# sidiso/surfh

Measured on AMD Instinct MI355X. Metric: CG-iterations/sec (forward+adjoint) on 251x251x4000 cube, higher is better.
Workload: dtype f32 (storage and accumulation; products as 2-piece fp16 splits -- 3 products per fp32 product, 1 on the far tails of the spectral response -- on the 16-bit matrix cores, in the spectral-blur GEMM and in the DFT passes)

## Files before the change

include/surfh_amd.h:

```cpp
#ifndef SURFH_AMD_H
#define SURFH_AMD_H

#include <stdint.h>

#ifdef __cplusplus
extern "C" {
#endif

typedef struct surfh_plan surfh_plan;

typedef struct {
    int32_t wslice_start, wslice_stop;
    int32_t n_pointings;
    int32_t n_slit;
    int32_t n_lambda_out;
    int32_t n_alpha_out;
    int32_t srf;
    int32_t na, nb;
    int32_t alpha0;
    int32_t n_alpha_slit;
    int32_t n_beta_slit;
    const int32_t *slit_beta0;
    const double *slit_weights;
    const int32_t *grid_i0;
// ... 130 lines not shown

int surfh_profile_enable(surfh_plan *plan, int32_t on);
int surfh_profile_filter(surfh_plan *plan, const char *prefix);
int32_t surfh_profile_count(surfh_plan *plan);
int surfh_profile_get(surfh_plan *plan, int32_t i, const char **name, int64_t *launches, double *ms);
int surfh_profile_reset(surfh_plan *plan);

int64_t surfh_debug_copy(surfh_plan *plan, const char *which, float *out, int64_t capacity);
int surfh_debug_dims(surfh_plan *plan, const char *which, int64_t dims[4]);

int surfh_gemm_selftest(int32_t device, int32_t M, int32_t N, int32_t K, int32_t split_k,
                        const float *A, const float *B, float *C);
int surfh_gemm_selftest_ksteps(int64_t near_far[2]);
int32_t surfh_klist_classify(const float *B, int32_t n, int32_t k, int64_t ldb, int32_t perm_p, int32_t perm_lin,
                             int32_t *records, int64_t capacity);

typedef struct surfh_tst surfh_tst;
int surfh_tst_create(int32_t n_alpha, int32_t n_beta, int32_t n_lambda, int32_t n_templates, const double *templates,
                     const int32_t *voxels, int64_t n_voxels, const float *S, int32_t device, surfh_tst **out);
int surfh_tst_destroy(surfh_tst *t);
int surfh_tst_forward(surfh_tst *t, const float *maps, float *cube);
int surfh_tst_adjoint(surfh_tst *t, const float *cube, float *maps);
int surfh_tst_fwadj(surfh_tst *t, const float *maps, float *out);
const char *surfh_tst_last_error(void);

int surfh_shepard(int32_t n_seg, const int64_t *pt_off, const float *pt_alpha, const float *pt_lambda,
                  const float *pt_value, const int32_t *n_alpha, const int32_t *n_lambda, int32_t separable,
                  const float *q_alpha, const float *q_lambda, const float *inv_alpha_res, const float *inv_lambda_res,
                  float p, float alpha, float pixel_cutoff, float epsilon, float *out, int32_t *neighbours,
                  int32_t device_ptrs, void *stream, float *kernel_ms);
// ... 14 lines not shown
```

surfh_amd/_lib.py:

```python
from __future__ import annotations

import ctypes as C
import os

import numpy as np

_HERE = os.path.dirname(os.path.abspath(__file__))
LIB_PATH = os.path.join(_HERE, "libsurfh_amd.so")

c_float_p = C.POINTER(C.c_float)
c_double_p = C.POINTER(C.c_double)
c_int32_p = C.POINTER(C.c_int32)
CG_CALLBACK = C.CFUNCTYPE(C.c_int, C.c_void_p, C.c_int32, c_double_p, c_float_p)
c_uint8_p = C.POINTER(C.c_uint8)


class ChannelDesc(C.Structure):
    _fields_ = [
        ("wslice_start", C.c_int32), ("wslice_stop", C.c_int32),
        ("n_pointings", C.c_int32), ("n_slit", C.c_int32), ("n_lambda_out", C.c_int32),
        ("n_alpha_out", C.c_int32), ("srf", C.c_int32), ("na", C.c_int32), ("nb", C.c_int32),
        ("alpha0", C.c_int32), ("n_alpha_slit", C.c_int32), ("n_beta_slit", C.c_int32),
        ("slit_beta0", c_int32_p), ("slit_weights", c_double_p),
        ("grid_i0", c_int32_p), ("grid_i1", c_int32_p), ("grid_y0", c_double_p), ("grid_y1", c_double_p),
# ... 13 lines not shown
        ("exact", C.c_int32),
    ]


EXPORTS = [
    "surfh_last_error", "surfh_version", "surfh_plan_create", "surfh_plan_destroy", "surfh_isize", "surfh_osize",
    "surfh_stream", "surfh_forward", "surfh_adjoint", "surfh_adjoint_ref", "surfh_fwadj", "surfh_forward_dev",
    "surfh_adjoint_dev", "surfh_adjoint_ref_dev", "surfh_fwadj_dev", "surfh_wct_forward", "surfh_wct_adjoint",
    "surfh_wct_fwadj", "surfh_wct_expsol", "surfh_tst_create", "surfh_tst_destroy", "surfh_tst_forward",
    "surfh_tst_adjoint", "surfh_tst_fwadj", "surfh_tst_last_error", "surfh_cg", "surfh_cg_cb", "surfh_mmmg", "surfh_mmmg_huber", "surfh_huber_prior_dev", "surfh_huber_curv_dev", "surfh_mmmg_huber_vox", "surfh_huber_vox_prior_dev", "surfh_huber_vox_curv_dev", "surfh_mmmg_huber_planes", "surfh_huber_planes_prior_dev", "surfh_huber_planes_curv_dev", "surfh_cg_planes", "surfh_mmmg_planes", "surfh_cg_planes_cb", "surfh_mmmg_planes_cb", "surfh_cg_planes_begin_dev", "surfh_cg_planes_step_dev", "surfh_cg_planes_rr", "surfh_maps_to_cube", "surfh_cube_to_maps", "surfh_normal_dev",
    "surfh_prior_add_dev", "surfh_spec_supported", "surfh_spec_size", "surfh_to_spec_dev", "surfh_from_spec_dev", "surfh_forward_spec_dev",
    "surfh_adjoint_spec_dev", "surfh_normal_spec_dev", "surfh_prior_spec_add_dev", "surfh_set_prior", "surfh_set_data_weights", "surfh_set_data_weights_dev", "surfh_has_data_weights", "surfh_dot_dev", "surfh_cg_step_dev", "surfh_cg_dir_dev", "surfh_cg_iter_dev", "surfh_residual_dev",
    "surfh_cg_begin_dev", "surfh_cg_iter_nosync_dev", "surfh_cg_xupdate_nosync_dev", "surfh_cg_refresh_nosync_dev", "surfh_cg_trace",
    "surfh_profile_enable", "surfh_profile_filter", "surfh_profile_count", "surfh_profile_get", "surfh_profile_reset", "surfh_debug_copy",
    "surfh_debug_dims", "surfh_gemm_selftest", "surfh_gemm_selftest_ksteps", "surfh_klist_classify",
    "surfh_shepard", "surfh_shepard_last_error", "surfh_spectral_median", "surfh_nmf_cd", "surfh_templates_last_error",
]

_lib = None


def load():
    global _lib
    if _lib is not None:
        return _lib
    if not os.path.exists(LIB_PATH):
        raise RuntimeError(f"{LIB_PATH} not found: run `python -c 'import __graft_entry__ as g; g.build()'` "
                           "(the HIP path has no CPU fallback)")
    L = C.CDLL(LIB_PATH)
    vp = C.c_void_p
# ... 65 lines not shown
    L.surfh_cg_iter_nosync_dev.argtypes = [vp, vp, vp, vp, vp, C.c_int64]
    L.surfh_cg_xupdate_nosync_dev.argtypes = [vp, vp, vp, vp, C.c_int64]
    L.surfh_cg_refresh_nosync_dev.argtypes = [vp, vp, vp, vp, vp, C.c_int64]
    L.surfh_cg_trace.argtypes = [vp, c_double_p, C.c_int32]; L.surfh_cg_trace.restype = C.c_int32
    L.surfh_profile_enable.argtypes = [vp, C.c_int32]
    L.surfh_profile_filter.argtypes = [vp, C.c_char_p]
    L.surfh_profile_count.argtypes = [vp]; L.surfh_profile_count.restype = C.c_int32
    L.surfh_profile_get.argtypes = [vp, C.c_int32, C.POINTER(C.c_char_p), C.POINTER(C.c_int64), c_double_p]
    L.surfh_profile_reset.argtypes = [vp]
    L.surfh_debug_copy.argtypes = [vp, C.c_char_p, c_float_p, C.c_int64]; L.surfh_debug_copy.restype = C.c_int64
    L.surfh_debug_dims.argtypes = [vp, C.c_char_p, C.POINTER(C.c_int64)]
    L.surfh_gemm_selftest.argtypes = [C.c_int32] * 5 + [c_float_p, c_float_p, c_float_p]
    L.surfh_gemm_selftest_ksteps.argtypes = [C.POINTER(C.c_int64)]
    L.surfh_klist_classify.argtypes = [c_float_p, C.c_int32, C.c_int32, C.c_int64, C.c_int32, C.c_int32, C.POINTER(C.c_int32), C.c_int64]
    L.surfh_klist_classify.restype = C.c_int32
    L.surfh_shepard.argtypes = [C.c_int32, C.POINTER(C.c_int64), vp, vp, vp, c_int32_p, c_int32_p, C.c_int32, vp, vp,
                                c_float_p, c_float_p, C.c_float, C.c_float, C.c_float, C.c_float, vp, vp, C.c_int32, vp,
                                c_float_p]
    L.surfh_shepard_last_error.restype = C.c_char_p
    L.surfh_spectral_median.argtypes = [c_float_p, c_float_p, C.c_int64, C.c_int64, C.c_int32, C.c_int32, C.c_int32]
    L.surfh_nmf_cd.argtypes = [c_float_p, C.c_int64, C.c_int64, C.c_int32, c_int32_p, c_float_p, c_float_p, C.c_int32,
                               C.c_double, c_int32_p, c_double_p, c_double_p, c_double_p, C.c_int32, c_float_p]
    L.surfh_templates_last_error.restype = C.c_char_p
    _lib = L
    return L


def check(rc: int, exc=RuntimeError):
    if rc != 0:
        raise exc(load().surfh_last_error().decode("utf-8", "replace"))
# ... 82 lines not shown
```

surfh_amd/csrc/dft_h2.h:

```cpp
#pragma once
#include <hip/hip_runtime.h>

constexpr int DFT_H2_KT = 8;
constexpr size_t DFT_H2_IMAGE_HALFS = (size_t)2 * 2 * DFT_H2_KT * 128 * 16;

struct DftH2Args {
    int kind = 0;
    const float *src = nullptr;
    long ldb = 0, sB = 0;
    int Kn = 0;
    float *dst = nullptr;
    long ldc = 0, sC = 0;
    float e[4] = {1.f, 0.f, 0.f, 1.f};
    float e_alt[4] = {1.f, 0.f, 0.f, 1.f};
    int Rn = 0, rvalid = 0;
    int KP = 0;
    int N = 0, batch = 1;
    const float *mhat = nullptr, *tpl = nullptr;
    int T = 0, LP = 0;
    long PL = 0, KBP = 0;
    int mix_l0 = 0;
    float mhat_self = 1.f, mhat_pair = 1.f;
    int mix_Nb = 0;
    const int *vlist = nullptr;
    int nvalid = 0;
    const int *ktab = nullptr, *rtab = nullptr;
    int tabLP = 0;
};

struct DftH2AdjMix {
    const float *hsrc = nullptr;
    long ldh = 0, sH = 0;
    const float *tpl = nullptr;
    int T = 0, LPt = 0;
    float *mpart = nullptr;
    int nslot = 0;
    int kt0 = 0;
    float out_self = 1.f, out_pair = 1.f;
    int Nb = 0;
    const float *prior_src = nullptr;
// ... 12 lines not shown
```

surfh_amd/csrc/dft_h2.hip:

```cpp
#include "dft_h2.h"
#include "lds_attr.h"
#include <cmath>
#include <cstring>

typedef float f32x16 __attribute__((ext_vector_type(16)));
typedef float f32x2 __attribute__((ext_vector_type(2)));
typedef unsigned u32x2 __attribute__((ext_vector_type(2)));
typedef _Float16 f16x8 __attribute__((ext_vector_type(8)));

#ifndef H2_EXP
#define H2_EXP 0
#endif

namespace {

constexpr int BK = 16, RS = 16;
constexpr int PIECE = 128 * RS;
constexpr int KT = DFT_H2_KT;
constexpr int IMG_HALFS = (int)DFT_H2_IMAGE_HALFS;
constexpr int MIX_ROWS = 256;
constexpr size_t LDS_IMG = (size_t)IMG_HALFS * 2;
constexpr size_t LDS_MIX = (size_t)2 * MIX_ROWS * 2 * sizeof(float4);
#ifndef H2_WAVES
#define H2_WAVES 8
// ... 173 lines not shown

    if (MIX) {
        if (ntw > 0) {
            const int t0_ = NWAVES * s0 + wave;
            const int kb0 = g.batch > 1 ? t0_ / tilesX : ((t0_ % tilesX) * TNW) / g.LP;
            H2_MIXTAB(kb0);
        }
    }
    __syncthreads();
    if (ntw <= 0) return;

    const int *vl = g.vlist;
#define H2_RT(vt_) (vl ? NWAVES * vl[(vt_) >> 3] + ((vt_) & 7) : (vt_))
    int vt = NWAVES * s0 + wave;
    const int vtend = vt + NWAVES * ntw;
    int tile = H2_RT(vt);
    int e = 0, en = 0;

    H2_LSETUP(tile);
    H2_LOAD(0);
    H2_FSETUP(tile);
    H2_FOLD(0);
    {
        int p;
        H2_MAXEXP(p);
        e = E_TARGET - p;
    }
    split8h(x0, e, c0h, c0l);
    split8h(x1, e, c1h, c1l);
    H2_LOAD(1);
    while (true) {
        asm volatile("" : "+v"(hv));
#pragma unroll
        for (int i = 0; i < 4; ++i)
#pragma unroll
            for (int r = 0; r < 16; ++r) acc1[i][r] = acc2[i][r] = 0.f;
        const bool more = vt + NWAVES < vtend;
        const int next = more ? H2_RT(vt + NWAVES) : tile;
        const int chunk_ = g.tabLP ? (int)(((long)(tile % tilesX) * TNW % g.tabLP) >> 7) : 0;
        const int nkt = g.ktab ? g.ktab[chunk_] : nk;
        const int mtn = g.rtab ? (g.rtab[chunk_] + 31) / 32 : 4;
        for (int kt = 0; kt + 1 < nkt; ++kt) {
            H2_MFMA(0, kt, acc1, c0h, c0l);
            H2_FOLD(kt + 1);
            int p;
            H2_MAXEXP(p);
            const bool need = p + e > E_LIMIT;
            en = need ? E_TARGET - p : e;
            const int d = en - e;
            if (kt + 2 < nkt) {
                H2_LOAD(kt + 2);
            } else if (more) {
                H2_LSETUP(next);
                H2_LOAD(0);
            }
// ... 45 lines not shown
                            __builtin_amdgcn_raw_buffer_store_b64(__builtin_bit_cast(u32x2, v2), W0, (int)lo, (int)sk0, 0);
                        } else {
                            __builtin_amdgcn_raw_buffer_store_b32(__float_as_uint(e0 * a1 + e1 * a2), W0, (int)lo, (int)sk0, 0);
                            if (row >= 1 && 2 * row != g.Rn)
                                __builtin_amdgcn_raw_buffer_store_b32(__float_as_uint(e2 * a1 + e3 * a2), W0, (int)lm, (int)sm0, 0);
                        }
                    }
                    const unsigned st = ((r & 3) == 3) ? 5u * ldc4 : ldc4;
                    sk0 += st; sm0 -= st;
                }
            }
        }
        if (!more) break;
        e = en;
        tile = next;
        vt += NWAVES;
    }
}


__device__ __forceinline__ float wave_max(float m) {
#define H2_DPPMAX(ctrl_) m = fmaxf(m, __builtin_bit_cast(float, __builtin_amdgcn_update_dpp(0, __builtin_bit_cast(int, m), ctrl_, 0xF, 0xF, false)))
    H2_DPPMAX(0xB1);
    H2_DPPMAX(0x4E);
    H2_DPPMAX(0x141);
    H2_DPPMAX(0x140);
#undef H2_DPPMAX
    unsigned u = __float_as_uint(m);
    auto s16 = __builtin_amdgcn_permlane16_swap(u, u, false, false);
    m = fmaxf(m, fmaxf(__uint_as_float(s16[0]), __uint_as_float(s16[1])));
    u = __float_as_uint(m);
    auto s32 = __builtin_amdgcn_permlane32_swap(u, u, false, false);
// ... 342 lines not shown
    const int mix_rows = g.Kn > g.KP ? g.Kn : g.KP;
    if (g.mhat && (g.kind != 0 || g.LP % 128 || g.T < 1 || g.T > 4 || mix_rows > MIX_ROWS || !g.tpl)) return (int)hipErrorInvalidValue;
    static int cus_of[64] = {0};
    int dev = 0;
    if (hipGetDevice(&dev) != hipSuccess || dev < 0 || dev >= 64) return (int)hipErrorInvalidDevice;
    if (!cus_of[dev]) {
        int cus = 0;
        if (hipDeviceGetAttribute(&cus, hipDeviceAttributeMultiprocessorCount, dev) != hipSuccess) return (int)hipErrorInvalidDevice;
        cus_of[dev] = cus;
    }
    const int tnw = g.kind == 0 ? 16 : 32;
    long NT = (long)(g.N / tnw) * g.batch;
    long NS = (NT + NWAVES - 1) / NWAVES;
    if (NS >= 2147483647L / NWAVES) return (int)hipErrorInvalidValue;
    if ((g.ktab || g.rtab) && (g.tabLP < 128 || g.tabLP % 128)) return (int)hipErrorInvalidValue;
    if (g.vlist) {
        if (NT % NWAVES || g.nvalid < 1 || g.nvalid > NS) return (int)hipErrorInvalidValue;
        NS = g.nvalid;
        NT = NS * NWAVES;
    }
    dim3 grid((unsigned)(NS < cus_of[dev] ? NS : cus_of[dev]));
    const uint4 *im = reinterpret_cast<const uint4 *>(img);
    static unsigned long long d0 = 0, d1 = 0, d2 = 0, d3 = 0;
    if (g.mhat) {
        if (int e = ensure_dynamic_lds(dft_h2_kernel<0, true>, LDS_IMG + LDS_MIX, d3)) return e;
        hipLaunchKernelGGL((dft_h2_kernel<0, true>), grid, dim3(NTHREADS), LDS_IMG + LDS_MIX, stream, g, im, kA, (int)NS, NT);
    } else if (g.kind == 0) {
        if (int e = ensure_dynamic_lds(dft_h2_kernel<0, false>, LDS_IMG, d0)) return e;
        hipLaunchKernelGGL((dft_h2_kernel<0, false>), grid, dim3(NTHREADS), LDS_IMG, stream, g, im, kA, (int)NS, NT);
    } else if (g.kind == 1) {
// ... 60 lines not shown
```

surfh_amd/csrc/plan.hip:

```cpp
#include <hip/hip_runtime.h>

#include <algorithm>
#include <array>
#include <cfloat>
#include <cmath>
#include <cstdarg>
#include <cstdio>
#include <cstring>
#include <map>
#include <string>
#include <vector>

#include "../../include/surfh_amd.h"
#include "dft_h2.h"
#include "dft_ct.h"
#include "gemm_f32.h"
#include "kernels.h"

namespace {

thread_local std::string g_err;

int fail(const char *fmt, ...) {
    char buf[1024];
// ... 109 lines not shown
    unsigned short *h2img = nullptr;
    bool ct = false, ilv = false;
    DftCtPlan ctA, ctB;
    int ax_a = 0, ax_b = 0;
    int a_lo = 0, a_hi = 0, b_lo = 0, b_hi = 0;
    float *ycol_adj = nullptr;
    const float *spec_in = nullptr;
    float *spec_out = nullptr;
    const float *spec_prior_src = nullptr;
    float spec_mu = 1.f, spec_prior_mu = 0.f;
    float *adjmix_part = nullptr;
    int *otf_vlist = nullptr, *otf_kbstart = nullptr;
    int otf_nvalid = 0;
    int *otf_tabs = nullptr;
    float *ycol_mix = nullptr;
    int h2kA[3] = {0, 0, 0};
    float *io_x = nullptr, *io_y = nullptr, *io_cube = nullptr, *hth = nullptr, *mhat2 = nullptr;
    float *gcube = nullptr;
    std::vector<Channel> ch;
    long isize = 0, osize = 0;
    float *dw = nullptr, *dwy = nullptr;
    float *cg_x = nullptr, *cg_r = nullptr, *cg_d = nullptr, *cg_q = nullptr, *cg_b = nullptr, *cg_y = nullptr, *cg_qm = nullptr, *cg_dd = nullptr;
    float *cg_hg = nullptr;
    double *dscal = nullptr, *dscratch = nullptr;
    double *cg_hist = nullptr;
    int cg_hist_n = 0;
    double *pl_sc = nullptr;
    double *pl_hsc = nullptr;
    float *pl_x = nullptr;
    double pl_mu = 1.0, pl_mu_reg = 0.0;
// ... 601 lines not shown
        Prof pr(p, "gemm_dft_cols_inv");
        LAUNCH_OK(gemm32(p, p->stream, g));
    }
    GemmArgs h;
    h.A0 = p->GiT; h.lda = 2 * p->KBP;
    h.B0 = p->ycol; h.B1 = p->ycol + (long)p->NAP * p->KBP * LP; h.ksplitB = p->KBP; h.ldb = LP; h.sB = p->KBP * LP;
    h.C = dst; h.ldc = p->NAP * LP; h.sC = LP;
    h.M = p->NBP; h.N = (int)LP; h.K = 2 * p->KBP; h.batch = p->NAP;
    {
        Prof pr(p, "gemm_dft_rows_inv");
        LAUNCH_OK(gemm32(p, p->stream, h));
    }
    return 0;
}

int otf_support(surfh_plan *p, const surfh_config *cfg) {
    const bool on = [] { const char *e = getenv("SURFH_OTF_SUPPORT"); return !(e && e[0] == '0'); }();
    if (cfg->exact & 2) return 0;
    if (!on || !cfg->sotf || !p->ilv || p->T < 1 || !p->fuse_mix || p->LP % 128) return 0;
    const int nkb = p->Nb / 2 + 1, nch = (int)(p->LP / 128);
    std::vector<int> bmax(nch, -1), amaxk(nch, -1);
    std::vector<double> km(nkb), kam(p->Na);
    for (int l = 0; l < p->Lown; ++l) {
        if (p->planes[l] < 0) continue;
        std::fill(km.begin(), km.end(), 0.0);
        std::fill(kam.begin(), kam.end(), 0.0);
        double amax = 0.0;
        const double *pl = cfg->sotf + (size_t)p->planes[l] * p->Na * nkb * 2;
        for (int a = 0; a < p->Na; ++a)
            for (int k = 0; k < nkb; ++k) {
                const double re = pl[((size_t)a * nkb + k) * 2], im = pl[((size_t)a * nkb + k) * 2 + 1], m2 = re * re + im * im;
                if (m2 > km[k]) km[k] = m2;
                if (m2 > kam[a]) kam[a] = m2;
            }
        for (int k = 0; k < nkb; ++k) amax = std::max(amax, km[k]);
        const double thr = amax * std::ldexp(1.0, -48);
        int b = -1;
        for (int k = 0; k < nkb; ++k)
            if (km[k] > thr) b = k;
        bmax[l / 128] = std::max(bmax[l / 128], b);
        int af = -1;
        for (int a = 0; a < p->Na; ++a)
            if (kam[a] > thr) af = std::max(af, std::min(a, p->Na - a));
        amaxk[l / 128] = std::max(amaxk[l / 128], af);
    }
    std::vector<int> vlist, kbstart(nkb + 1, 0);
    for (int kb = 0; kb < nkb; ++kb) {
        kbstart[kb] = (int)vlist.size();
        for (int j = 0; j < nch; ++j)
            if (kb <= bmax[j]) vlist.push_back(kb * nch + j);
    }
    kbstart[nkb] = (int)vlist.size();
    if (vlist.empty() || (long)vlist.size() == (long)nkb * nch) return 0;
    const size_t nyc = (size_t)2 * p->NAP * p->KBP * p->LP;
    if (dev_upload(&p->otf_vlist, vlist) || dev_upload(&p->otf_kbstart, kbstart) || dev_alloc(&p->ycol_mix, nyc)) return 1;
    if (hipMemset(p->ycol_mix, 0, nyc * sizeof(float)) != hipSuccess) return fail("memset failed");
    p->otf_nvalid = (int)vlist.size();
    std::vector<int> tabs((size_t)(p->ct ? 4 : 3) * nch);
    for (int j = 0; j < nch; ++j) {
        if (p->ct) {
            const int ja = (std::max(amaxk[j], 0) + p->ctA.R - 1) / p->ctA.R, jb = (std::max(bmax[j], 0) + p->ctB.R - 1) / p->ctB.R;
            tabs[j] = std::min(std::max(ja / 16 + 1, 2), p->ctA.KT);
            tabs[nch + j] = std::min(std::max(jb / 16 + 1, 2), p->ctB.KT);
            tabs[2 * nch + j] = bmax[j];
            tabs[3 * nch + j] = amaxk[j];
            continue;
        }
        tabs[j] = std::min(std::max((amaxk[j] + 16) / 16, 2), p->KPa / 16);
        tabs[nch + j] = std::min(std::max((bmax[j] + 16) / 16, 2), p->KPb / 16);
        tabs[2 * nch + j] = bmax[j] + 1;
    }
    const bool ranges = [] { const char *e = getenv("SURFH_OTF_RANGES"); return !(e && e[0] == '0'); }();
    if (ranges && dev_upload(&p->otf_tabs, tabs)) return 1;
    return 0;
}

int rfft2_lam_h2(surfh_plan *p, const float *src, float *dst, float *madj = nullptr, bool acols = false, int which = 3) {
    const long LP = p->LP;
    const int ha = p->Na / 2 + 1, hb = p->Nb / 2 + 1;
    const bool sub = acols && p->ycol_adj && p->a_hi > p->a_lo;
    float *const yc = sub ? p->ycol_adj : p->ycol;
    const int a0 = sub ? p->a_lo : 0, na = sub ? p->a_hi - p->a_lo : p->Na;
    DftH2Args g;
    g.kind = 1; g.src = src + (long)a0 * LP; g.ldb = p->NAP * LP; g.Kn = p->Nb;
    g.dst = yc + 2 * (long)a0 * LP; g.ldc = 2 * p->NAP * LP; g.e[0] = 1.f; g.e[3] = -1.f; g.rvalid = hb;
    g.KP = p->KPb; g.N = (int)(na * LP);
    if (madj && p->otf_vlist && p->ycol_mix && p->otf_tabs) { g.rtab = p->otf_tabs + 2 * (LP / 128); g.tabLP = (int)LP; }
    if (which & 1) {
        Prof pr(p, "dft_h2_rows_fwd");
        LAUNCH_OK(launch_dft_h2(p->stream, g, p->h2img + 2 * DFT_H2_IMAGE_HALFS, p->h2kA[2]));
    }
    if (!(which & 2)) return 0;
    DftH2Args h;
    h.kind = 0; h.src = yc; h.ldb = 2 * LP; h.sB = 2 * p->NAP * LP; h.Kn = p->Na;
    h.dst = dst; h.ldc = 2 * p->KBP * LP; h.sC = 2 * LP; h.Rn = p->Na; h.rvalid = ha;
    h.KP = p->KPa; h.N = (int)LP; h.batch = hb;
    h.e[0] = 1.f; h.e[1] = 1.f; h.e[2] = 1.f; h.e[3] = -1.f;
    h.e_alt[0] = 1.f; h.e_alt[1] = -1.f; h.e_alt[2] = 1.f; h.e_alt[3] = 1.f;
// ... 24 lines not shown
int irfft2_lam_h2(surfh_plan *p, const float *src, float *dst, bool mix, bool acols = false, int which = 3) {
    const long LP = p->LP;
    const int ha = p->Na / 2 + 1, hb = p->Nb / 2 + 1;
    DftH2Args g;
    g.kind = 0; g.src = src; g.ldb = 2 * p->KBP * LP; g.Kn = p->Na;
    g.dst = p->ycol; g.ldc = 2 * p->KBP * LP; g.Rn = p->Na; g.rvalid = ha;
    g.KP = p->KPa; g.N = (int)(hb * LP);
    g.e[0] = 1.f; g.e[1] = -1.f; g.e[2] = 1.f; g.e[3] = 1.f;
    g.e_alt[0] = 1.f; g.e_alt[1] = 1.f; g.e_alt[2] = 1.f; g.e_alt[3] = -1.f;
    if (mix) { g.mhat = p->mhat; g.tpl = p->tpl; g.T = p->T; g.LP = (int)p->LP; g.PL = p->PL; g.KBP = p->KBP; }
    if (mix && p->spec_in) { g.mhat = p->spec_in; g.mhat_self = 1.f; g.mhat_pair = 0.70710678118654752f; g.mix_Nb = p->Nb; }
    const bool supp = mix && p->otf_vlist && p->ycol_mix && p->adjmix_part;
    float *const yc = supp ? p->ycol_mix : p->ycol;
    if (supp) { g.vlist = p->otf_vlist; g.nvalid = p->otf_nvalid; g.dst = yc; }
    if (supp && p->otf_tabs) { g.ktab = p->otf_tabs; g.tabLP = (int)LP; }
    if (which & 2) {
        Prof pr(p, mix ? "dft_h2_cols_inv_mix" : "dft_h2_cols_inv");
        LAUNCH_OK(launch_dft_h2(p->stream, g, p->h2img, p->h2kA[0]));
    }
    if (!(which & 1)) return 0;
    const bool sub = acols && p->a_hi > p->a_lo;
    const int a0 = sub ? p->a_lo : 0, na = sub ? p->a_hi - p->a_lo : p->Na;
    DftH2Args h;
    h.kind = 2; h.src = yc + (long)a0 * 2 * p->KBP * LP; h.ldb = 2 * LP; h.sB = 2 * p->KBP * LP;
    h.dst = dst + (long)a0 * LP; h.ldc = p->NAP * LP; h.sC = LP;
    h.e[0] = 1.f; h.e[1] = -1.f; h.e[2] = 1.f; h.e[3] = 1.f; h.Rn = p->Nb; h.rvalid = hb;
    h.KP = p->KPb; h.N = (int)LP; h.batch = na;
    if (supp && p->otf_tabs) { h.ktab = p->otf_tabs + LP / 128; h.tabLP = (int)LP; }
    {
        Prof pr(p, "dft_h2_rows_inv");
        LAUNCH_OK(launch_dft_h2(p->stream, h, p->h2img + DFT_H2_IMAGE_HALFS, p->h2kA[1]));
    }
    return 0;
}

int rfft2_lam_ct(surfh_plan *p, const float *src, float *dst, bool acols = false, bool lists = false, int which = 3) {
    const long LP = p->LP;
    const int hb = p->Nb / 2 + 1;
    const bool sub = acols && p->ycol_adj && p->a_hi > p->a_lo;
    float *const yc = sub ? p->ycol_adj : p->ycol;
    const int a0 = sub ? p->a_lo : 0, na = sub ? p->a_hi - p->a_lo : p->Na;
    DftCtArgs g;
    g.R = p->ctB.R; g.M = p->ctB.M; g.loader = DFT_CT_PLAIN; g.epi = DFT_CT_HSEP; g.sgn = -1.f;
// ... 410 lines not shown
int surfh_version(void) { return 100; }

int surfh_plan_destroy(surfh_plan *p) {
    if (!p) return 0;
    hipSetDevice(p->dev);
    if (p->stream) hipStreamSynchronize(p->stream);
    for (float *v : {p->sotf, p->tpl, p->mhat, p->spec, p->ycol, p->cube, p->ycol_maps, p->maps_pad, p->Fi, p->Gi, p->Gf,
                     p->Ff, p->GiT, p->GfT, p->Cma, p->Sma, p->Gc, p->Gs, p->Cf, p->Sf, p->io_cube, p->hth, p->mhat2, p->gcube, p->io_x, p->io_y, p->cg_x, p->cg_r, p->cg_d, p->cg_q, p->cg_b, p->cg_y, p->cg_qm, p->cg_dd, p->cg_hg})
        hipFree(v);
    hipFree(p->h2img);
    if (p->ctB.img != p->ctA.img) dft_ct_plan_destroy(&p->ctB);
    else p->ctB = DftCtPlan();
    dft_ct_plan_destroy(&p->ctA);
    hipFree(p->adjmix_part);
    hipFree(p->otf_vlist);
    hipFree(p->otf_kbstart);
    hipFree(p->otf_tabs);
    hipFree(p->ycol_mix);
    hipFree(p->ycol_adj);
    hipFree(p->dscal);
    hipFree(p->dscratch);
    hipFree(p->cg_hist);
    hipFree(p->pl_sc);
    hipFree(p->pl_hsc);
    for (float *v : p->pn_v) hipFree(v);
    hipFree(p->dw);
    hipFree(p->dwy);
    hipFree(p->pn_sc);
    hipFree(p->pn_part);
    for (auto &c : p->ch) {
// ... 100 lines not shown

    {
        const char *eh = getenv("SURFH_DFT_H2"), *ec = getenv("SURFH_DFT_CT"), *ed = getenv("SURFH_DFT_DENSE");
        const bool h2_on = !(eh && eh[0] == '0'), ct_on = !(ec && ec[0] == '0');
        auto axis = [&](int n) {
            if (h2_on && dft_h2_supported(n, n, p->NAP, p->KBP, p->LP)) return 1;
            if (ct_on && dft_ct_factor(n, nullptr, nullptr)) return 2;
            return 0;
        };
        p->ax_a = axis(p->Na);
        p->ax_b = axis(p->Nb);
        p->ilv = !cfg->verify && !(ed && ed[0] == '1') && p->LP % 128 == 0 && p->ax_a && p->ax_b;
        if (!p->ilv) p->ax_a = p->ax_b = 0;
        p->h2 = p->ilv && p->ax_a == 1 && p->ax_b == 1;
        p->ct = p->ilv && !p->h2;
    }
    {
        const int nkb = p->Nb / 2 + 1;
        const size_t nsp = (size_t)2 * p->PL * LP;
        if (dev_alloc(&p->sotf, nsp)) return bail(1);
        if (hipMemset(p->sotf, 0, nsp * sizeof(float)) != hipSuccess) return bail(fail("memset failed"));
        std::vector<float> row((size_t)2 * p->KBP * LP);
        for (int a = 0; a < p->Na; ++a) {
            std::fill(row.begin(), row.end(), 0.f);
            for (int l = 0; l < p->Lown; ++l) {
                if (p->planes[l] < 0) continue;
                const double *src = cfg->sotf ? cfg->sotf + ((size_t)p->planes[l] * p->Na + a) * nkb * 2 : nullptr;
                for (int k = 0; k < nkb; ++k) {
                    const float vr = src ? (float)src[2 * k] : 1.f, vi = src ? (float)src[2 * k + 1] : 0.f;
                    if (p->ilv) {
// ... 234 lines not shown
                    size_t n = 1;
                    while (n < (size_t)SCATTER_G && r + n < h.rows.size() && h.dst[r + n] == h.dst[r + n - 1] + p->LP) ++n;
                    runs.push_back({r, n});
                    r += n;
                }
                if (upload_groups(h, runs, &mask, &c.adjT, SCATTER_G, &ranges)) return bail(1);
            }
            c.adjT_host = HostEll();
            if (dev_upload(&c.adjT.rmw, mask) || dev_upload(&c.adjT.rng, ranges)) return bail(1);
            c.adjT.t.rng = c.adjT.rng;
            const char *ea = getenv("SURFH_SCATTER_RMW_ALL");
            if (!(ea && ea[0] == '1')) c.adjT.t.rmw = c.adjT.rmw;
            c.adjT.host_dst.clear();
            c.adjT.host_dst.shrink_to_fit();
        }
        if (exact_ok && !p->ch.empty()) {
            const size_t ncube = (size_t)p->NBP * p->NAP * p->LP;
            if (dev_alloc(&p->gcube, ncube)) return bail(1);
            if (hipMemset(p->gcube, 0, ncube * sizeof(float)) != hipSuccess) return bail(fail("memset failed"));
        } else {
            for (auto &c : p->ch) {
                c.adjT.t.rng = nullptr;
                c.adjT.g.rng = nullptr;
            }
        }
    }
    if (dev_alloc(&p->io_x, (size_t)p->isize) || dev_alloc(&p->io_y, (size_t)p->osize) || dev_alloc(&p->cg_y, (size_t)p->osize) ||
        dev_alloc(&p->dscal, 16) || dev_alloc(&p->dscratch, std::max((size_t)1024, launch_huber_vox_scratch_doubles())))
        return bail(1);
    if (hipDeviceSynchronize() != hipSuccess) return bail(fail("device error during plan creation: %s", hipGetErrorString(hipGetLastError())));
// ... 1241 lines not shown
            dims[0] = p->ch[c].LinP; dims[1] = p->ch[c].shift; dims[2] = p->ch[c].nbs; dims[3] = p->ch[c].Lin;
        } else {
            Channel &ch = p->ch[c];
            if (ch.Xs16) {
                if (launch_dequant_f16x2(p->stream, ch.Xs16, (long)ch.NP * ch.K, ch.bscale, ch.Xs, ch.NP, ch.K, ch.LinP,
                                         (ch.LinP + 1023) / 1024))
                    return fail("dequant launch failed");
                if (hipStreamSynchronize(p->stream) != hipSuccess) return fail("dequant failed");
            }
            *ptr = p->ch[c].Xs; dims[0] = p->ch[c].NP; dims[1] = p->ch[c].bsum ? 1 : p->ch[c].nbs; dims[2] = p->ch[c].LinP;
        }
    } else if (w == "range") {
        dims[0] = p->a_lo; dims[1] = p->a_hi; dims[2] = p->b_lo; dims[3] = p->b_hi;
    } else if (w == "otf") {
        dims[0] = p->otf_vlist ? p->otf_nvalid : (long)(p->Nb / 2 + 1) * (p->LP / 128); dims[1] = (long)(p->Nb / 2 + 1) * (p->LP / 128);
    } else if (w == "ksteps") {
        for (auto &c : p->ch)
            for (int i = 0; i < 4; ++i) dims[i] += c.ksteps[i];
        for (int i = 0; i < 4; ++i) dims[i] -= 1;
    } else if (w == "info") {
        dims[0] = p->lo; dims[1] = p->hi; dims[2] = p->Lown; dims[3] = (int64_t)p->segs.size();
    } else {
        return fail("unknown debug buffer '%s'", w.c_str());
    }
    return 0;
}

int surfh_debug_dims(surfh_plan *p, const char *which, int64_t dims[4]) {
    if (!p) return fail("null plan");
    const float *ptr;
// ... 16 lines not shown
    return n;
}

int32_t surfh_klist_classify(const float *B, int32_t n, int32_t k, int64_t ldb, int32_t perm_p, int32_t perm_lin, int32_t *records,
                             int64_t capacity) {
    if (!B || !records || n < 1 || k < 32 || k % 32 || ldb < k) return -fail("surfh_klist_classify: bad arguments");
    if (perm_p && ((perm_p != 1 && perm_p != 2 && perm_p != 4 && perm_p != 8) || perm_lin < 1 || perm_lin % (256 / perm_p) || n % perm_lin))
        return -fail("surfh_klist_classify: bad tile shape");
    std::vector<int> kl;
    int stride = 0;
    long nn = 0, nf = 0;
    build_klist(B, n, k, ldb, 0, 0, 1.0 / 256, 1.0 / 1024, &kl, &stride, &nn, &nf, perm_p, perm_lin);
    if ((int64_t)kl.size() > capacity) return -fail("surfh_klist_classify: capacity too small");
    std::memcpy(records, kl.data(), kl.size() * sizeof(int));
    return (int32_t)(kl.size() / (size_t)stride);
}

static long g_selftest_ksteps[2] = {0, 0};
int surfh_gemm_selftest_ksteps(int64_t near_far[2]) {
    near_far[0] = g_selftest_ksteps[0]; near_far[1] = g_selftest_ksteps[1];
    return 0;
}

int surfh_gemm_selftest(int32_t device, int32_t M, int32_t N, int32_t K, int32_t split_k, const float *A,
                        const float *B, float *C) {
    HIP_OK(hipSetDevice(device));
    float *dA = nullptr, *dB = nullptr, *dC = nullptr;
    const int sk = std::max(1, (int)split_k);
    HIP_OK(hipMalloc((void **)&dA, (size_t)M * K * 4));
    HIP_OK(hipMalloc((void **)&dB, (size_t)K * N * 4));
// ... 68 lines not shown
```

Baseline: 357.1.

## Tighten OTF support with per-tile k-step counts and skip dead spectral tiles

Computes the spectral OTF's alpha-frequency limit per (beta-frequency, 128-lane chunk) so each listed DFT tile runs only the MFMA k-steps it needs, instead of a per-chunk maximum. It also builds a map of live (alpha row, lambda chunk) tiles from the channels' touched footprint, and the h2 DFT kernel skips tiles that no channel observes in the adjoint column and row passes. This removes matrix-core work on zero or unobserved regions. It adds host-side precomputation, per-tile table lookups and skip loops in the kernel, and relies on the thresholded OTF support being accurate enough.

```diff
diff --git a/include/surfh_amd.h b/include/surfh_amd.h
--- a/include/surfh_amd.h
+++ b/include/surfh_amd.h
@@ -168,6 +168,9 @@
 int surfh_gemm_selftest_ksteps(int64_t near_far[2]);
 int32_t surfh_klist_classify(const float *B, int32_t n, int32_t k, int64_t ldb, int32_t perm_p, int32_t perm_lin,
                              int32_t *records, int64_t capacity);
+int32_t surfh_tight_otf_limits(const double *sotf, int32_t L, int32_t Na, int32_t Nb, int32_t *klim, int32_t *ksteps, int32_t *kept);
+int32_t surfh_tight_live_tiles(const uint8_t *touched, const int32_t *windows, int32_t n_channels, int32_t Na, int32_t Nb, int32_t LP,
+                               uint8_t *live);
 
 typedef struct surfh_tst surfh_tst;
 int surfh_tst_create(int32_t n_alpha, int32_t n_beta, int32_t n_lambda, int32_t n_templates, const double *templates,
diff --git a/surfh_amd/_lib.py b/surfh_amd/_lib.py
--- a/surfh_amd/_lib.py
+++ b/surfh_amd/_lib.py
@@ -51,6 +51,7 @@
     "surfh_cg_begin_dev", "surfh_cg_iter_nosync_dev", "surfh_cg_xupdate_nosync_dev", "surfh_cg_refresh_nosync_dev", "surfh_cg_trace",
     "surfh_profile_enable", "surfh_profile_filter", "surfh_profile_count", "surfh_profile_get", "surfh_profile_reset", "surfh_debug_copy",
     "surfh_debug_dims", "surfh_gemm_selftest", "surfh_gemm_selftest_ksteps", "surfh_klist_classify",
+    "surfh_tight_otf_limits", "surfh_tight_live_tiles",
     "surfh_shepard", "surfh_shepard_last_error", "surfh_spectral_median", "surfh_nmf_cd", "surfh_templates_last_error",
 ]
 
@@ -146,6 +147,10 @@
     L.surfh_gemm_selftest_ksteps.argtypes = [C.POINTER(C.c_int64)]
     L.surfh_klist_classify.argtypes = [c_float_p, C.c_int32, C.c_int32, C.c_int64, C.c_int32, C.c_int32, C.POINTER(C.c_int32), C.c_int64]
     L.surfh_klist_classify.restype = C.c_int32
+    L.surfh_tight_otf_limits.argtypes = [c_double_p, C.c_int32, C.c_int32, C.c_int32, c_int32_p, c_int32_p, c_int32_p]
+    L.surfh_tight_otf_limits.restype = C.c_int32
+    L.surfh_tight_live_tiles.argtypes = [C.POINTER(C.c_uint8), c_int32_p, C.c_int32, C.c_int32, C.c_int32, C.c_int32, C.POINTER(C.c_uint8)]
+    L.surfh_tight_live_tiles.restype = C.c_int32
     L.surfh_shepard.argtypes = [C.c_int32, C.POINTER(C.c_int64), vp, vp, vp, c_int32_p, c_int32_p, C.c_int32, vp, vp,
                                 c_float_p, c_float_p, C.c_float, C.c_float, C.c_float, C.c_float, vp, vp, C.c_int32, vp,
                                 c_float_p]
diff --git a/surfh_amd/csrc/dft_h2.h b/surfh_amd/csrc/dft_h2.h
--- a/surfh_amd/csrc/dft_h2.h
+++ b/surfh_amd/csrc/dft_h2.h
@@ -24,6 +24,9 @@
     int mix_Nb = 0;
     const int *vlist = nullptr;
     int nvalid = 0;
+    const int *vkt = nullptr;
+    const unsigned char *live = nullptr;
+    int liveLP = 0;
     const int *ktab = nullptr, *rtab = nullptr;
     int tabLP = 0;
 };
diff --git a/surfh_amd/csrc/dft_h2.hip b/surfh_amd/csrc/dft_h2.hip
--- a/surfh_amd/csrc/dft_h2.hip
+++ b/surfh_amd/csrc/dft_h2.hip
@@ -211,6 +211,12 @@
 #define H2_RT(vt_) (vl ? NWAVES * vl[(vt_) >> 3] + ((vt_) & 7) : (vt_))
     int vt = NWAVES * s0 + wave;
     const int vtend = vt + NWAVES * ntw;
+    const int lper = MIX || !g.live ? 0 : g.liveLP / TNW;
+#define H2_DEAD(t_) (!g.live[(long)((t_) / lper) * (g.liveLP >> 7) + ((((t_) % lper) * TNW) >> 7)])
+    if (lper) {
+        while (vt < vtend && H2_DEAD(H2_RT(vt))) vt += NWAVES;
+        if (vt >= vtend) return;
+    }
     int tile = H2_RT(vt);
     int e = 0, en = 0;
 
@@ -232,10 +238,13 @@
         for (int i = 0; i < 4; ++i)
 #pragma unroll
             for (int r = 0; r < 16; ++r) acc1[i][r] = acc2[i][r] = 0.f;
-        const bool more = vt + NWAVES < vtend;
-        const int next = more ? H2_RT(vt + NWAVES) : tile;
+        int nvt = vt + NWAVES;
+        if (lper)
+            while (nvt < vtend && H2_DEAD(H2_RT(nvt))) nvt += NWAVES;
+        const bool more = nvt < vtend;
+        const int next = more ? H2_RT(nvt) : tile;
         const int chunk_ = g.tabLP ? (int)(((long)(tile % tilesX) * TNW % g.tabLP) >> 7) : 0;
-        const int nkt = g.ktab ? g.ktab[chunk_] : nk;
+        const int nkt = g.vkt ? g.vkt[vt >> 3] : g.ktab ? g.ktab[chunk_] : nk;
         const int mtn = g.rtab ? (g.rtab[chunk_] + 31) / 32 : 4;
         for (int kt = 0; kt + 1 < nkt; ++kt) {
             H2_MFMA(0, kt, acc1, c0h, c0l);
@@ -311,8 +320,9 @@
         if (!more) break;
         e = en;
         tile = next;
-        vt += NWAVES;
-    }
+        vt = nvt;
+    }
+#undef H2_DEAD
 }
 
 
@@ -685,6 +695,8 @@
     long NS = (NT + NWAVES - 1) / NWAVES;
     if (NS >= 2147483647L / NWAVES) return (int)hipErrorInvalidValue;
     if ((g.ktab || g.rtab) && (g.tabLP < 128 || g.tabLP % 128)) return (int)hipErrorInvalidValue;
+    if (g.vkt && !g.vlist) return (int)hipErrorInvalidValue;
+    if (g.live && (g.mhat || g.kind == 0 || g.liveLP < 128 || g.liveLP % 128 || g.N % g.liveLP)) return (int)hipErrorInvalidValue;
     if (g.vlist) {
         if (NT % NWAVES || g.nvalid < 1 || g.nvalid > NS) return (int)hipErrorInvalidValue;
         NS = g.nvalid;
diff --git a/surfh_amd/csrc/plan.hip b/surfh_amd/csrc/plan.hip
--- a/surfh_amd/csrc/plan.hip
+++ b/surfh_amd/csrc/plan.hip
@@ -147,6 +147,10 @@
     int otf_nvalid = 0;
     int *otf_tabs = nullptr;
     float *ycol_mix = nullptr;
+    bool tight = false;
+    int *otf_vkt = nullptr;
+    unsigned char *live = nullptr;
+    long tight_stats[4] = {0, 0, 0, 0};
     int h2kA[3] = {0, 0, 0};
     float *io_x = nullptr, *io_y = nullptr, *io_cube = nullptr, *hth = nullptr, *mhat2 = nullptr;
     float *gcube = nullptr;
@@ -778,41 +782,72 @@
     return 0;
 }
 
+struct OtfLimits {
+    std::vector<int> bmax, amaxk, amk;
+};
+void otf_limits(const double *sotf, const int *planes, int Lown, int Na, int nkb, int nch, OtfLimits *o) {
+    o->bmax.assign(nch, -1);
+    o->amaxk.assign(nch, -1);
+    o->amk.assign((size_t)nkb * nch, -1);
+    std::vector<double> km(nkb);
+    for (int l = 0; l < Lown && l / 128 < nch; ++l) {
+        const int src = planes ? planes[l] : l;
+        if (src < 0) continue;
+        std::fill(km.begin(), km.end(), 0.0);
+        double amax = 0.0;
+        const double *pl = sotf + (size_t)src * Na * nkb * 2;
+        for (int a = 0; a < Na; ++a)
+            for (int k = 0; k < nkb; ++k) {
+                const double re = pl[((size_t)a * nkb + k) * 2], im = pl[((size_t)a * nkb + k) * 2 + 1], m2 = re * re + im * im;
+                if (m2 > km[k]) km[k] = m2;
+            }
+        for (int k = 0; k < nkb; ++k) amax = std::max(amax, km[k]);
+        const double thr = amax * std::ldexp(1.0, -48);
+        const int j = l / 128;
+        for (int k = 0; k < nkb; ++k) {
+            if (!(km[k] > thr)) continue;
+            o->bmax[j] = std::max(o->bmax[j], k);
+            int af = -1;
+            for (int a = 0; a < Na; ++a) {
+                const double re = pl[((size_t)a * nkb + k) * 2], im = pl[((size_t)a * nkb + k) * 2 + 1];
+                if (re * re + im * im > thr) af = std::max(af, std::min(a, Na - a));
+            }
+            o->amk[(size_t)k * nch + j] = std::max(o->amk[(size_t)k * nch + j], af);
+            o->amaxk[j] = std::max(o->amaxk[j], af);
+        }
+    }
+}
+int ksteps_of_limit(int amax, int KP) { return std::min(std::max((amax + 16) / 16, 2), KP / 16); }
+
+void live_tiles(const std::vector<const uint8_t *> &touched, const std::vector<int> &w0, const std::vector<int> &wn, int Na, int Nb,
+                long pitch, int nch, std::vector<unsigned char> *live) {
+    live->assign((size_t)Na * nch, 0);
+    for (size_t c = 0; c < touched.size(); ++c)
+        for (int a = 0; a < Na; ++a) {
+            bool any = false;
+            for (int b = 0; b < Nb && !any; ++b) any = touched[c][(size_t)b * pitch + a] != 0;
+            if (!any) continue;
+            for (int j = 0; j < nch; ++j)
+                if (w0[c] < 128 * (j + 1) && w0[c] + wn[c] > 128 * j) (*live)[(size_t)a * nch + j] = 1;
+        }
+}
+
 int otf_support(surfh_plan *p, const surfh_config *cfg) {
     const bool on = [] { const char *e = getenv("SURFH_OTF_SUPPORT"); return !(e && e[0] == '0'); }();
     if (cfg->exact & 2) return 0;
     if (!on || !cfg->sotf || !p->ilv || p->T < 1 || !p->fuse_mix || p->LP % 128) return 0;
     const int nkb = p->Nb / 2 + 1, nch = (int)(p->LP / 128);
-    std::vector<int> bmax(nch, -1), amaxk(nch, -1);
-    std::vector<double> km(nkb), kam(p->Na);
-    for (int l = 0; l < p->Lown; ++l) {
-        if (p->planes[l] < 0) continue;
-        std::fill(km.begin(), km.end(), 0.0);
-        std::fill(kam.begin(), kam.end(), 0.0);
-        double amax = 0.0;
-        const double *pl = cfg->sotf + (size_t)p->planes[l] * p->Na * nkb * 2;
-        for (int a = 0; a < p->Na; ++a)
-            for (int k = 0; k < nkb; ++k) {
-                const double re = pl[((size_t)a * nkb + k) * 2], im = pl[((size_t)a * nkb + k) * 2 + 1], m2 = re * re + im * im;
-                if (m2 > km[k]) km[k] = m2;
-                if (m2 > kam[a]) kam[a] = m2;
-            }
-        for (int k = 0; k < nkb; ++k) amax = std::max(amax, km[k]);
-        const double thr = amax * std::ldexp(1.0, -48);
-        int b = -1;
-        for (int k = 0; k < nkb; ++k)
-            if (km[k] > thr) b = k;
-        bmax[l / 128] = std::max(bmax[l / 128], b);
-        int af = -1;
-        for (int a = 0; a < p->Na; ++a)
-            if (kam[a] > thr) af = std::max(af, std::min(a, p->Na - a));
-        amaxk[l / 128] = std::max(amaxk[l / 128], af);
-    }
-    std::vector<int> vlist, kbstart(nkb + 1, 0);
+    OtfLimits lim;
+    otf_limits(cfg->sotf, p->planes.data(), p->Lown, p->Na, nkb, nch, &lim);
+    const std::vector<int> &bmax = lim.bmax, &amaxk = lim.amaxk;
+    std::vector<int> vlist, vkt, kbstart(nkb + 1, 0);
     for (int kb = 0; kb < nkb; ++kb) {
         kbstart[kb] = (int)vlist.size();
         for (int j = 0; j < nch; ++j)
-            if (kb <= bmax[j]) vlist.push_back(kb * nch + j);
+            if (kb <= bmax[j]) {
+                vlist.push_back(kb * nch + j);
+                vkt.push_back(ksteps_of_limit(lim.amk[(size_t)kb * nch + j], p->KPa));
+            }
     }
     kbstart[nkb] = (int)vlist.size();
     if (vlist.empty() || (long)vlist.size() == (long)nkb * nch) return 0;
@@ -830,22 +865,32 @@
             tabs[3 * nch + j] = amaxk[j];
             continue;
         }
-        tabs[j] = std::min(std::max((amaxk[j] + 16) / 16, 2), p->KPa / 16);
-        tabs[nch + j] = std::min(std::max((bmax[j] + 16) / 16, 2), p->KPb / 16);
+        tabs[j] = ksteps_of_limit(amaxk[j], p->KPa);
+        tabs[nch + j] = ksteps_of_limit(bmax[j], p->KPb);
         tabs[2 * nch + j] = bmax[j] + 1;
     }
     const bool ranges = [] { const char *e = getenv("SURFH_OTF_RANGES"); return !(e && e[0] == '0'); }();
     if (ranges && dev_upload(&p->otf_tabs, tabs)) return 1;
+    if (p->tight && p->h2) {
+        if (dev_upload(&p->otf_vkt, vkt)) return 1;
+        for (size_t i = 0; i < vlist.size(); ++i) {
+            p->tight_stats[0] += vkt[i];
+            p->tight_stats[1] += tabs[vlist[i] % nch];
+        }
+    }
     return 0;
 }
 
 int rfft2_lam_h2(surfh_plan *p, const float *src, float *dst, float *madj = nullptr, bool acols = false, int which = 3) {
     const long LP = p->LP;
     const int ha = p->Na / 2 + 1, hb = p->Nb / 2 + 1;
-    const bool sub = acols && p->ycol_adj && p->a_hi > p->a_lo;
+    const bool listed = p->live && p->gcube;
+    const bool tiles = acols && listed && src == p->gcube;
+    const bool sub = acols && p->ycol_adj && p->a_hi > p->a_lo && (tiles || !listed);
     float *const yc = sub ? p->ycol_adj : p->ycol;
     const int a0 = sub ? p->a_lo : 0, na = sub ? p->a_hi - p->a_lo : p->Na;
     DftH2Args g;
+    if (tiles && sub) { g.live = p->live + (long)a0 * (LP / 128); g.liveLP = (int)LP; }
     g.kind = 1; g.src = src + (long)a0 * LP; g.ldb = p->NAP * LP; g.Kn = p->Nb;
     g.dst = yc + 2 * (long)a0 * LP; g.ldc = 2 * p->NAP * LP; g.e[0] = 1.f; g.e[3] = -1.f; g.rvalid = hb;
     g.KP = p->KPb; g.N = (int)(na * LP);
@@ -900,6 +945,7 @@
     float *const yc = supp ? p->ycol_mix : p->ycol;
     if (supp) { g.vlist = p->otf_vlist; g.nvalid = p->otf_nvalid; g.dst = yc; }
     if (supp && p->otf_tabs) { g.ktab = p->otf_tabs; g.tabLP = (int)LP; }
+    if (supp && p->otf_vkt) g.vkt = p->otf_vkt;
     if (which & 2) {
         Prof pr(p, mix ? "dft_h2_cols_inv_mix" : "dft_h2_cols_inv");
         LAUNCH_OK(launch_dft_h2(p->stream, g, p->h2img, p->h2kA[0]));
@@ -913,6 +959,7 @@
     h.e[0] = 1.f; h.e[1] = -1.f; h.e[2] = 1.f; h.e[3] = 1.f; h.Rn = p->Nb; h.rvalid = hb;
     h.KP = p->KPb; h.N = (int)LP; h.batch = na;
     if (supp && p->otf_tabs) { h.ktab = p->otf_tabs + LP / 128; h.tabLP = (int)LP; }
+    if (acols && p->live) { h.live = p->live + (long)a0 * (LP / 128); h.liveLP = (int)LP; }
     {
         Prof pr(p, "dft_h2_rows_inv");
         LAUNCH_OK(launch_dft_h2(p->stream, h, p->h2img + DFT_H2_IMAGE_HALFS, p->h2kA[1]));
@@ -1353,6 +1400,8 @@
     dft_ct_plan_destroy(&p->ctA);
     hipFree(p->adjmix_part);
     hipFree(p->otf_vlist);
+    hipFree(p->otf_vkt);
+    hipFree(p->live);
     hipFree(p->otf_kbstart);
     hipFree(p->otf_tabs);
     hipFree(p->ycol_mix);
@@ -1483,6 +1532,8 @@
         if (!p->ilv) p->ax_a = p->ax_b = 0;
         p->h2 = p->ilv && p->ax_a == 1 && p->ax_b == 1;
         p->ct = p->ilv && !p->h2;
+        const char *etl = getenv("SURFH_TIGHT_LISTS");
+        p->tight = p->h2 && !(cfg->exact & 2) && !(etl && etl[0] == '0');
     }
     {
         const int nkb = p->Nb / 2 + 1;
@@ -1747,6 +1798,22 @@
             c.adjT.host_dst.clear();
             c.adjT.host_dst.shrink_to_fit();
         }
+        if (p->tight && !p->verify && !p->ch.empty() && p->LP % 128 == 0) {
+            std::vector<const uint8_t *> tp;
+            std::vector<int> w0, wn;
+            for (size_t ci = 0; ci < p->ch.size(); ++ci) {
+                tp.push_back(touched[ci].data());
+                w0.push_back(p->ch[ci].ws0a);
+                wn.push_back(p->ch[ci].nlam);
+            }
+            std::vector<unsigned char> live;
+            live_tiles(tp, w0, wn, p->Na, p->Nb, p->NAP, (int)(p->LP / 128), &live);
+            if (dev_upload(&p->live, live)) return bail(1);
+            const long nch = p->LP / 128;
+            for (long a = p->a_lo; a < p->a_hi; ++a)
+                for (long j = 0; j < nch; ++j) p->tight_stats[2] += live[(size_t)(a * nch + j)];
+            p->tight_stats[3] = (long)(p->a_hi - p->a_lo) * nch;
+        }
         if (exact_ok && !p->ch.empty()) {
             const size_t ncube = (size_t)p->NBP * p->NAP * p->LP;
             if (dev_alloc(&p->gcube, ncube)) return bail(1);
@@ -3018,6 +3085,8 @@
         dims[0] = p->a_lo; dims[1] = p->a_hi; dims[2] = p->b_lo; dims[3] = p->b_hi;
     } else if (w == "otf") {
         dims[0] = p->otf_vlist ? p->otf_nvalid : (long)(p->Nb / 2 + 1) * (p->LP / 128); dims[1] = (long)(p->Nb / 2 + 1) * (p->LP / 128);
+    } else if (w == "tight") {
+        for (int i = 0; i < 4; ++i) dims[i] = p->tight_stats[i];
     } else if (w == "ksteps") {
         for (auto &c : p->ch)
             for (int i = 0; i < 4; ++i) dims[i] += c.ksteps[i];
@@ -3064,6 +3133,41 @@
     if ((int64_t)kl.size() > capacity) return -fail("surfh_klist_classify: capacity too small");
     std::memcpy(records, kl.data(), kl.size() * sizeof(int));
     return (int32_t)(kl.size() / (size_t)stride);
+}
+
+int32_t surfh_tight_otf_limits(const double *sotf, int32_t L, int32_t Na, int32_t Nb, int32_t *klim, int32_t *ksteps, int32_t *kept) {
+    if (!sotf || !klim || !ksteps || !kept || L < 1 || Na < 34 || Nb < 2) return -fail("surfh_tight_otf_limits: bad arguments");
+    const int nkb = Nb / 2 + 1, nch = (L + 127) / 128, KPa = (Na / 2 + 1 + 15) / 16 * 16;
+    OtfLimits lim;
+    otf_limits(sotf, nullptr, L, Na, nkb, nch, &lim);
+    int32_t n = 0;
+    for (int kb = 0; kb < nkb; ++kb)
+        for (int j = 0; j < nch; ++j) {
+            const size_t i = (size_t)kb * nch + j;
+            klim[i] = lim.amk[i];
+            ksteps[i] = ksteps_of_limit(lim.amk[i], KPa);
+            kept[i] = kb <= lim.bmax[j];
+            n += kept[i];
+        }
+    return n == nkb * nch ? 0 : n;
+}
+
+int32_t surfh_tight_live_tiles(const uint8_t *touched, const int32_t *windows, int32_t n_channels, int32_t Na, int32_t Nb, int32_t LP,
+                               uint8_t *live) {
+    if (!touched || !windows || !live || n_channels < 1 || Na < 1 || Nb < 1 || LP < 128 || LP % 128) return -fail("surfh_tight_live_tiles: bad arguments");
+    std::vector<const uint8_t *> tp;
+    std::vector<int> w0, wn;
+    for (int c = 0; c < n_channels; ++c) {
+        tp.push_back(touched + (size_t)c * Na * Nb);
+        w0.push_back(windows[2 * c]);
+        wn.push_back(windows[2 * c + 1]);
+    }
+    std::vector<unsigned char> lv;
+    live_tiles(tp, w0, wn, Na, Nb, Na, LP / 128, &lv);
+    std::memcpy(live, lv.data(), lv.size());
+    int32_t n = 0;
+    for (unsigned char v : lv) n += v;
+    return n;
 }
 
 static long g_selftest_ksteps[2] = {0, 0};
```

Result: faster. 362.2 (median of 6 runs) (+1.4%).
